# MinghanLi/UniVS

Hardware: AMD Instinct MI355X
Metric: frames/sec per node, 720p T=5 clip, Swin-T 100Q; mask-logit max-abs-err (higher is better)
Workload: dtype f32; 1 GPU; BASELINE config 2: Swin-T UniVS, T=5 @ 720p (736x1280 padded), 100 queries, first clip (no prompt queries); one clip per GPU; frames_per_clip=5, queries=100, parallelism=clip-replicas x1

## Files before the change

### univs_amd/build.py

```python
import os
import shutil
import subprocess
import sys

HERE = os.path.dirname(os.path.abspath(__file__))
CSRC = os.path.join(HERE, "csrc")
LIB = os.path.join(HERE, "libunivs_hip.so")
SOURCES = ["capi.hip", "msda_fwd.hip", "msda_tiled2.hip", "msda_strips.hip", "msda_heads.hip", "msda_bwd.hip", "msda_prepare.hip", "mask_decode.hip", "linear_split.hip", "linear_f16x3.hip", "gemm_f16x3_stream.hip", "gemm_f16x3_tile.hip", "mlp_f16x3.hip", "small_linear.hip", "cross_attn.hip", "window_attn.hip", "window_attn_f16.hip", "resample.hip", "semantic_extract.hip", "layer_norm.hip", "group_norm.hip", "softmax.hip", "proca_attn.hip", "prompt_sampler.hip", "transpose.hip", "mask_stats.hip", "image_post.hip", "video_post.hip", "pair_count.hip", "vss_count.hip", "davis_count.hip", "vis_overlap.hip", "pvos_count.hip", "semantic_decode.hip"]
HEADERS = [os.path.join(CSRC, "common.h"), os.path.join(CSRC, "msda_common.h"), os.path.join(CSRC, "msda_geometry.h"), os.path.join(CSRC, "msda_dev.h"), os.path.join(CSRC, "msda_window_geom.h"), os.path.join(CSRC, "msda_strips_geom.h"), os.path.join(CSRC, "msda_heads_geom.h"), os.path.join(CSRC, "config.h"), os.path.join(CSRC, "window_attn.h"), os.path.join(CSRC, "f16x3.h"), os.path.join(CSRC, "gemm_plan.h"), os.path.join(CSRC, "resample_taps.h"),
           os.path.join(CSRC, "mask_post.h"), os.path.join(CSRC, "count_core.h"), os.path.join(CSRC, "launchers.h"), os.path.join(CSRC, "xattn_merge.h"), os.path.join(CSRC, "skinny_gemm_f32.h"), os.path.join(HERE, "..", "include", "univs_hip.h"),
           os.path.join(HERE, "..", "include", "univs_eval_hip.h"), os.path.join(HERE, "..", "include", "univs_fused_hip.h"),
           os.path.join(HERE, "..", "include", "univs_pvos_hip.h"), os.path.join(HERE, "..", "include", "univs_semantic_hip.h")]


def _hipcc():
    for c in (os.environ.get("HIPCC"), shutil.which("hipcc"), "/opt/rocm/bin/hipcc"):
        if c and os.path.exists(c):
            return c
    raise RuntimeError("hipcc not found (set HIPCC or install ROCm)")


def needs_build():
    if not os.path.exists(LIB):
        return True
    t = os.path.getmtime(LIB)
    deps = [os.path.join(CSRC, s) for s in SOURCES if os.path.exists(os.path.join(CSRC, s))] + HEADERS
    return any(os.path.getmtime(d) > t for d in deps)


def _flags(defines=()):
    return ["--offload-arch=gfx950", "-O3", "-std=c++17", "-fPIC", "-fno-gpu-rdc", "-Wall", "-Wno-unused-function",
            "-I", os.path.join(HERE, "..", "include"), *[f"-D{d}" for d in defines]]


def build(force=False, verbose=True, lib=LIB, defines=(), tag=""):
    if not force and not defines and not needs_build():
        return lib
    from concurrent.futures import ThreadPoolExecutor
    objdir = os.path.join(HERE, "_obj" + tag)
    os.makedirs(objdir, exist_ok=True)
    hipcc = _hipcc()
    hdr_t = max(os.path.getmtime(h) for h in HEADERS)
    srcs = [s for s in SOURCES if os.path.exists(os.path.join(CSRC, s))]

    def compile_one(s):
        src, obj = os.path.join(CSRC, s), os.path.join(objdir, s.replace(".hip", ".o"))
        if not force and os.path.exists(obj) and os.path.getmtime(obj) > max(os.path.getmtime(src), hdr_t):
            return obj
        cmd = [hipcc, *_flags(defines), "-c", src, "-o", obj]
        if verbose:
            print("[univs_amd.build]", " ".join(cmd), file=sys.stderr, flush=True)
        subprocess.run(cmd, check=True)
        return obj

    with ThreadPoolExecutor(max_workers=min(8, os.cpu_count() or 2)) as ex:
        objs = list(ex.map(compile_one, srcs))
    cmd = [hipcc, "--offload-arch=gfx950", "-fPIC", "-shared", "-fno-gpu-rdc", *objs, "-o", lib + ".tmp"]
    if verbose:
        print("[univs_amd.build]", " ".join(cmd), file=sys.stderr, flush=True)
    subprocess.run(cmd, check=True)
    os.replace(lib + ".tmp", lib)
# ... 25 lines not shown
```

### univs_amd/csrc/capi.hip

```cpp
#include <stdarg.h>
#include <string.h>

#include <mutex>

#include "../../include/univs_eval_hip.h"
#include "../../include/univs_fused_hip.h"
#include "../../include/univs_pvos_hip.h"
#include "../../include/univs_semantic_hip.h"
#include "common.h"
#include "config.h"
#include "launchers.h"

namespace univs {

static thread_local char g_err[512] = "";

void set_error(const char* fmt, ...) {
  va_list ap;
  va_start(ap, fmt);
  vsnprintf(g_err, sizeof(g_err), fmt, ap);
  va_end(ap);
}

static void report(const char* name, const char* fmt, va_list ap) {
// ... 45 lines not shown
UnivsConfig config() {
  std::lock_guard<std::mutex> lock(g_cfg_mu);
  return g_cfg;
}
static thread_local int g_msda_last = 0;
static thread_local int g_msda_gen = 0;

static int make_levels(const Entry& e, const int64_t* shapes, const int64_t* starts, int L, int S, LevelTable* lv) {
  if (L < 1 || L > UNIVS_MAX_LEVELS) return e.invalid("num_levels=%d outside [1,%d]", L, UNIVS_MAX_LEVELS);
  if (!shapes || !starts) return e.invalid("spatial_shapes / level_start_index must be host pointers, got NULL");
  int64_t run = 0;
  for (int l = 0; l < L; ++l) {
    const int64_t H = shapes[2 * l], W = shapes[2 * l + 1], st = starts[l];
    if (H <= 0 || W <= 0 || st != run || st + H * W > (int64_t)S)
      return e.invalid("level %d (H=%lld, W=%lld, start=%lld) is inconsistent: expected start=%lld, value length S=%d", l, (long long)H,
                       (long long)W, (long long)st, (long long)run, S);
    run += H * W;
    lv->H[l] = (int)H;
    lv->W[l] = (int)W;
    lv->start[l] = (int)st;
  }
  if (run != (int64_t)S) return e.invalid("the %d levels hold %lld tokens but value has S=%d", L, (long long)run, S);
  for (int l = L; l < UNIVS_MAX_LEVELS; ++l) lv->H[l] = lv->W[l] = lv->start[l] = 0;
  return UNIVS_OK;
}

template <class F>
static int linear_entry(const Entry& e, long long M, int N, int K, int act, const float* residual, bool ptrs_ok, bool resident, F&& launch) {
  if (M < 0 || N < 0 || K < 1 || act < 0 || act > 2 || (act != 0 && residual))
    return e.invalid("bad arguments M=%lld N=%d K=%d act=%d%s", M, N, K, act,
                     (act != 0 && residual) ? " (an activation and a residual exclude each other)" : "");
  if (M == 0 || N == 0) return UNIVS_OK;
  if (!ptrs_ok) return e.null_pointer();
  const int rc = launch(residual ? 3 : act);
  return resident ? e.launched(rc, "shape M=%lld N=%d K=%d (or alignment) is not covered", M, N, K)
                  : e.covered(rc, "shape M=%lld N=%d K=%d (or alignment) is not covered", M, N, K);
}
template <class F>
static int linear_blocked_entry(const Entry& e, long long M, int N, int K, int rows_per_batch, int col_block, bool ptrs_ok, F&& launch) {
  if (M < 0 || N < 1 || K < 1 || rows_per_batch < 1 || col_block < 4 || col_block % 4 != 0 || N % col_block != 0 ||
      (M % rows_per_batch) != 0)
    return e.invalid("bad arguments M=%lld N=%d K=%d rows_per_batch=%d col_block=%d", M, N, K, rows_per_batch, col_block);
  if (M == 0) return UNIVS_OK;
  if (!ptrs_ok) return e.null_pointer();
  return e.launched(launch(), "shape M=%lld N=%d K=%d (or alignment) is not covered (K == 256, M >= 2048)", M, N, K);
}
template <class F>
static int conv_entry(const Entry& e, const char* covers, int T, int Cin, int Cout, int H, int W, bool ptrs_ok, F&& launch) {
  if (T < 0 || Cin < 1 || Cout < 0 || H < 0 || W < 0) return e.invalid("bad dimensions T=%d Cin=%d Cout=%d H=%d W=%d", T, Cin, Cout, H, W);
  if (T == 0 || Cout == 0 || H == 0 || W == 0) return UNIVS_OK;
  if (!ptrs_ok) return e.null_pointer();
  return e.covered(launch(), "T=%d Cin=%d Cout=%d H=%d W=%d not covered (%s)", T, Cin, Cout, H, W, covers);
}

}

using namespace univs;

extern "C" {

const char* univs_version(void) { return "univs_hip 0.1.0 gfx950"; }
const char* univs_last_error(void) { return g_err; }

int univs_configure(const UnivsConfig* cfg) {
  UnivsConfig c = {};
  if (cfg) {
    if (cfg->size < (int)(2 * sizeof(int)) || cfg->size > (int)sizeof(UnivsConfig))
      return invalid_argument(__func__, "UnivsConfig.size=%d (this library: %d)", cfg->size, (int)sizeof(UnivsConfig));
    memcpy(&c, cfg, (size_t)cfg->size);
    if (c.msda_impl < 0 || c.msda_impl > 2 || c.mask_decode_impl < 0 || c.mask_decode_impl > 2 || c.msda_halo > 64 ||
        (c.mask_decode_ct != 0 && c.mask_decode_ct != 2 && c.mask_decode_ct != 4) ||
        (c.linear_terms != 0 && c.linear_terms != 3 && c.linear_terms != 6) || c.mask_decode_wave_tiles > 64)
      return invalid_argument(__func__, "msda_impl=%d mask_decode_impl=%d msda_halo=%d mask_decode_ct=%d linear_terms=%d out of range", c.msda_impl,
                              c.mask_decode_impl, c.msda_halo, c.mask_decode_ct, c.linear_terms);
  }
  c.size = (int)sizeof(UnivsConfig);
  std::lock_guard<std::mutex> lock(g_cfg_mu);
  g_cfg = c;
  return UNIVS_OK;
}

int univs_get_config(UnivsConfig* out) {
  if (!out) return invalid_argument(__func__, "NULL");
  *out = config();
  out->size = (int)sizeof(UnivsConfig);
  return UNIVS_OK;
}

int univs_msda_set_impl(int impl) {
  if (impl < 0 || impl > 2) return invalid_argument(__func__, "impl=%d not in {0,1,2}", impl);
  std::lock_guard<std::mutex> lock(g_cfg_mu);
  g_cfg.msda_impl = impl;
  return UNIVS_OK;
}

int univs_msda_last_impl(void) { return g_msda_last; }
int univs_msda_last_tiled_generation(void) { return g_msda_gen; }

int univs_linear_fused_f32(const float* x, const float* weight, const float* bias, const float* residual, long long M, int N,
                           int K, int act, float* y, void* stream) {
  const Entry e("univs_linear_fused_f32", stream);
  return linear_entry(e, M, N, K, act, residual, x && weight && y, true,
                      [&](int epi) { return linear_split_f32(x, weight, bias, residual, y, M, N, K, epi, e.st); });
}

int univs_presplit_weights_f32(const float* w, int N, int K, int conv, void* wp, float* winv, void* stream) {
  const Entry e("univs_presplit_weights_f32", stream);
  if (N < 0 || K < 32 || K % 32 != 0 || conv < 0 || conv > 2 || (conv == 1 && K % 9 != 0))
    return e.invalid("bad arguments N=%d K=%d mode=%d (K a multiple of 32; mode 1: K = 9 Cin)", N, K, conv);
  if (N == 0) return UNIVS_OK;
  if (!w || !wp || !winv || (reinterpret_cast<uintptr_t>(wp) & 15)) return e.invalid("NULL or unaligned pointer");
  return presplit_f16x3(w, N, K, conv == 1 ? K / 9 : 0, conv == 2 ? 1 : 0, wp, winv, e.st);
}

int univs_conv1x1_presplit_f32(const float* x, const void* wp, const float* winv, const float* bias, int T, int Cin, int Cout, int H,
                               int W, float* y, void* stream) {
  const Entry e("univs_conv1x1_presplit_f32", stream);
  return conv_entry(e, "Cin % 96 or % 128, Cout % 16, >= 4096 pixels", T, Cin, Cout, H, W, x && wp && winv && y,
                    [&] { return conv1x1_f16x3_f32(x, wp, winv, bias, y, T, Cin, Cout, H, W, e.st); });
}

long long univs_cross_attention_workspace(int L, int S, int N, int H) {
  if (L <= 0 || S <= 0 || N <= 0 || H <= 0) return 0;
  return (long long)cross_attention_workspace_floats(L, S, N, H);
}

int univs_cross_attention_f32(const float* q, const float* k, const float* v, const uint8_t* mask, int L, int S, int N, int H, int head_dim,
                              int ldq, int ldk, int ldv, float scale, float* workspace, float* out, void* stream) {
  return univs_cross_attention_flagged_f32(q, k, v, mask, nullptr, 0u, L, S, N, H, head_dim, ldq, ldk, ldv, scale, workspace, out, stream);
}

int univs_cross_attention_flagged_f32(const float* q, const float* k, const float* v, const uint8_t* mask, const uint32_t* mask_row_flags,
                                      uint32_t mask_generation, int L, int S, int N, int H, int head_dim, int ldq, int ldk, int ldv,
                                      float scale, float* workspace, float* out, void* stream) {
  const Entry e("univs_cross_attention_f32", stream);
  if (L < 0 || S < 1 || N < 0 || H < 1 || head_dim < 1) return e.invalid("bad dimensions L=%d S=%d N=%d H=%d head_dim=%d", L, S, N, H, head_dim);
  if (L == 0 || N == 0) return UNIVS_OK;
  if (!q || !k || !v || !workspace || !out || (mask_row_flags && !mask)) return e.invalid("NULL data pointer (row flags come with a mask)");
  return e.covered(cross_attention_f32(q, k, v, mask, mask_row_flags, mask_generation, L, S, N, H, head_dim, ldq, ldk, ldv, scale, workspace,
                                       out, e.st),
                   "L=%d S=%d N=%d H=%d head_dim=%d not covered (head_dim == 32, S >= 32, with a mask S %% 4 == 0, "
                   "N * H <= 65535, 16-byte aligned pointers)", L, S, N, H, head_dim);
}

int univs_mlp_presplit_f32(const float* x, const void* w1p, const float* w1inv, const float* b1, const void* w2p, const float* w2inv,
                           const float* b2, const float* residual, const float* ln_weight, const float* ln_bias, float ln_eps,
                           const float* post_ln_weight, const float* post_ln_bias, float post_ln_eps, const float* post_add,
                           long long post_add_rows, float* y2, long long M, int C, int Hd, int act, float* y, void* stream) {
  return univs_mlp_presplit_v2_f32(x, w1p, w1inv, b1, w2p, w2inv, b2, residual, 0, ln_weight, ln_bias, ln_eps, post_ln_weight, post_ln_bias,
                                   post_ln_eps, post_add, post_add_rows, y2, M, C, Hd, act, y, stream);
}

int univs_mlp_presplit_v2_f32(const float* x, const void* w1p, const float* w1inv, const float* b1, const void* w2p, const float* w2inv,
                              const float* b2, const float* residual, int flags, const float* ln_weight,
                              const float* ln_bias, float ln_eps, const float* post_ln_weight, const float* post_ln_bias, float post_ln_eps,
                              const float* post_add, long long post_add_rows, float* y2, long long M, int C, int Hd, int act, float* y,
                              void* stream) {
  const Entry e("univs_mlp_presplit_f32", stream);
  if (M < 0 || C < 1 || Hd < 1 || (act != 1 && act != 2)) return e.invalid("bad arguments M=%lld C=%d Hd=%d act=%d (1 ReLU, 2 GELU)", M, C, Hd, act);
  if (M == 0) return UNIVS_OK;
  if (!x || !w1p || !w1inv || !w2p || !w2inv || !y) return e.null_pointer();
  if ((flags & ~3) || ((flags & 1) && (residual || !ln_weight || x == y)) || ((flags & 2) && (!post_ln_weight || !y2 || post_add || (flags & 1))))
    return e.invalid("flags=%d: UNIVS_MLP_RESIDUAL_IS_NORMED_X needs ln_weight, no residual pointer and y distinct from x "
                     "(the normalised rows are parked in y); UNIVS_MLP_DUAL_OUTPUT needs post_ln_weight and y2, no post_add, and excludes the other",
                     flags);
  return e.covered(mlp_f16x3_f32(x, w1p, w1inv, b1, w2p, w2inv, b2, residual, ln_weight, ln_bias, ln_eps, post_ln_weight, post_ln_bias,
                                 post_ln_eps, post_add, post_add_rows, y2, y, M, C, Hd, act, flags, e.st),
                   "shape M=%lld C=%d Hd=%d (or alignment) is not covered (C in 96 / 128 / 192 / 256 / 384, Hd %% 32 == 0, M >= 2048)", M, C, Hd);
}

int univs_small_linear_presplit_f32(const float* x, const float* x_add, const void* wp, const float* winv, const float* bias, int n_w,
                                    int f_off, const float* residual, const float* ln_weight, const float* ln_bias, float ln_eps,
// ... 2 lines not shown
  if (M < 0 || N < 0 || K < 1 || n_w < 1 || f_off < 0 || f_off + N > n_w)
    return e.invalid("bad arguments M=%lld N=%d K=%d n_w=%d f_off=%d", M, N, K, n_w, f_off);
  if (M == 0 || N == 0) return UNIVS_OK;
  if (!x || !wp || !winv || !y || (ln_bias && !ln_weight)) return e.null_pointer();
  return e.covered(small_linear_f32(x, x_add, wp, winv, bias, n_w, f_off, residual, ln_weight, ln_bias, ln_eps, y, M, N, K, relu, add_features,
                                    out_T, e.st),
                   "M=%lld N=%d K=%d not covered (K %% 32 == 0, N %% 16 == 0, f_off %% 4 == 0, with a LayerNorm "
                   "N == 256, M <= 1 048 560, 16-byte aligned pointers)", M, N, K);
}

int univs_small_mlp_presplit_f32(const float* x, int stages, const void* const* wp, const float* const* winv, const float* const* bias,
                                 const int* relu, const float* in_ln_weight, const float* in_ln_bias, float in_ln_eps, float* x_normed,
                                 long long M, int out_T, float* y, void* stream) {
  const Entry e("univs_small_mlp_presplit_f32", stream);
  if (M < 0 || stages < 1 || stages > 3 || out_T < 0) return e.invalid("bad arguments M=%lld stages=%d out_T=%d", M, stages, out_T);
  if (M == 0) return UNIVS_OK;
  if (!x || !y || !wp || !winv || !bias || !relu) return e.invalid("NULL pointer");
  return e.covered(small_chain_f32(x, stages, wp, winv, bias, relu, in_ln_weight, in_ln_bias, in_ln_eps, x_normed, y, M, out_T, e.st),
                   "M=%lld not covered (M <= 1 048 560, out_T | M, 16-byte aligned pointers, x_normed / bias only with a LayerNorm)", M);
}

int univs_linear_presplit_f32(const float* x, const void* wp, const float* winv, const float* bias, const float* residual,
                              long long M, int N, int K, int act, float* y, void* stream) {
  const Entry e("univs_linear_presplit_f32", stream);
  return linear_entry(e, M, N, K, act, residual, x && wp && winv && y, false, [&](int epi) {
    int rc = UNIVS_ERR_NOT_IMPLEMENTED;
    if (config().linear_ablate != 6) rc = linear_f16x3_tile_f32(x, wp, winv, bias, residual, y, M, N, K, epi, e.st);
    if (rc == UNIVS_ERR_NOT_IMPLEMENTED) rc = linear_f16x3_stream_f32(x, wp, winv, bias, residual, y, M, N, K, epi, e.st);
    return rc;
  });
}

int univs_linear_resident_presplit_f32(const float* x, const void* wp, const float* winv, const float* bias, const float* residual,
                                       long long M, int N, int K, int act, float* y, void* stream) {
  const Entry e("univs_linear_resident_presplit_f32", stream);
  return linear_entry(e, M, N, K, act, residual, x && wp && winv && y, true, [&](int epi) {
    return linear_split_f32(x, static_cast<const float*>(wp), bias, residual, y, M, N, K, epi, e.st, 0, 0, winv);
  });
}

int univs_linear_blocked_presplit_f32(const float* x, const void* wp, const float* winv, const float* bias, long long M, int N, int K,
                                      int rows_per_batch, int col_block, float* y, void* stream) {
  const Entry e("univs_linear_blocked_presplit_f32", stream);
  return linear_blocked_entry(e, M, N, K, rows_per_batch, col_block, x && wp && winv && y, [&] {
    return linear_split_f32(x, static_cast<const float*>(wp), bias, nullptr, y, M, N, K, 4, e.st, rows_per_batch, col_block,
                            winv);
  });
}

int univs_conv3x3_presplit_f32(const float* x, const void* wp, const float* winv, int T, int Cin, int Cout, int H, int W,
                               float* y, void* stream) {
  const Entry e("univs_conv3x3_presplit_f32", stream);
  return conv_entry(e, "Cin % 128, Cout % 16, >= 4096 pixels", T, Cin, Cout, H, W, x && wp && winv && y,
                    [&] { return conv3x3_f16x3_f32(x, wp, winv, y, T, Cin, Cout, H, W, e.st); });
}

int univs_conv3x3_nhwc_presplit_f32(const float* x, const void* wp, const float* winv, int T, int Cin, int Cout, int H, int W,
                                    float* y, void* stream) {
  const Entry e("univs_conv3x3_nhwc_presplit_f32", stream);
  return conv_entry(e, "Cin % 128, Cout % 16, >= 4096 pixels", T, Cin, Cout, H, W, x && wp && winv && y,
                    [&] { return conv3x3_nhwc_f16x3_f32(x, wp, winv, y, T, Cin, Cout, H, W, e.st); });
}

int univs_conv1x1_fused_presplit_f32(const float* x, int channels_last, const float* affine, const void* wp, const float* winv,
                                     const float* bias, int T, int Cin, int Cout, int H, int W, float* y, void* stream) {
  const Entry e("univs_conv1x1_fused_presplit_f32", stream);
  return conv_entry(e, "Cin % 96 or % 128, Cout % 16, >= 4096 pixels; with an affine H W >= 256 and Cin <= 1024", T, Cin, Cout, H, W,
                    x && wp && winv && y,
                    [&] { return conv1x1_fused_f16x3_f32(x, channels_last, affine, wp, winv, bias, y, T, Cin, Cout, H, W, e.st); });
}

int univs_cross_attention_partials_f32(const float* q, const float* k, const float* v, const uint8_t* mask, const uint32_t* mask_row_flags,
                                       uint32_t mask_generation, int L, int S, int N, int H, int head_dim, int ldq, int ldk, int ldv,
                                       float scale, float* workspace, int* plan, void* stream) {
  const Entry e("univs_cross_attention_partials_f32", stream);
  if (!plan) return e.invalid("NULL plan (a host int)");
  *plan = 0;
  if (L < 0 || S < 1 || N < 0 || H < 1 || head_dim < 1) return e.invalid("bad dimensions L=%d S=%d N=%d H=%d head_dim=%d", L, S, N, H, head_dim);
  if (L == 0 || N == 0) return UNIVS_OK;
  if (!q || !k || !v || !workspace || (mask_row_flags && !mask)) return e.invalid("NULL data pointer (row flags come with a mask)");
  return e.covered(cross_attention_partials_f32(q, k, v, mask, mask_row_flags, mask_generation, L, S, N, H, head_dim, ldq, ldk, ldv, scale,
                                                workspace, plan, e.st),
                   "L=%d S=%d N=%d H=%d head_dim=%d not covered (head_dim == 32, S >= 32, with a mask S %% 4 == 0, "
                   "N * H <= 65535, 16-byte aligned pointers)", L, S, N, H, head_dim);
}

int univs_small_linear_merged_presplit_f32(const float* workspace, long long workspace_floats, int plan, int L, int N, int H, const void* wp,
                                           const float* winv, const float* bias, int n_w, int f_off, const float* residual,
                                           const float* ln_weight, const float* ln_bias, float ln_eps, int n_out, float* y, void* stream) {
  const Entry e("univs_small_linear_merged_presplit_f32", stream);
  const int nseg = plan & 0xffff, nqb = plan >> 16;
  if (L < 0 || N < 0 || H < 1 || n_out < 0 || n_w < 1 || f_off < 0 || f_off + n_out > n_w)
    return e.invalid("bad arguments L=%d N=%d H=%d n_out=%d n_w=%d f_off=%d", L, N, H, n_out, n_w, f_off);
  if (L == 0 || N == 0 || n_out == 0) return UNIVS_OK;
  if (plan <= 0 || nseg < 1 || nqb < 1 || nqb > 7) return e.invalid("plan=%d is not segments + 65536 * query blocks per wave (1 .. 7)", plan);
  const long long chunks = ((long long)L + 16 * nqb - 1) / (16 * nqb);
  const long long need = chunks * N * H * nseg * (16 * nqb) * 34;
  if (workspace_floats < need)
    return e.invalid("workspace of %lld floats, the plan %d of L=%d N=%d H=%d takes %lld", workspace_floats, plan, L, N, H, need);
  if (!workspace || !wp || !winv || !y || (ln_bias && !ln_weight)) return e.null_pointer();
  return e.covered(small_linear_merged_f32(workspace, plan, L, N, H, wp, winv, bias, n_w, f_off, residual, ln_weight, ln_bias, ln_eps, y,
                                           n_out, e.st),
                   "L=%d N=%d H=%d n_out=%d not covered (H <= 8, n_out %% 16 == 0, f_off %% 4 == 0, with a LayerNorm n_out == 256, "
                   "L N <= 1 048 560, 16-byte aligned pointers)", L, N, H, n_out);
}

int univs_patch_embed4_f32(const float* x, const float* weight, const float* bias, const float* ln_weight, const float* ln_bias, float ln_eps,
                           int T, int H, int W, int E, float* out, void* stream) {
  const Entry e("univs_patch_embed4_f32", stream);
  if (T < 0 || H < 0 || W < 0 || E < 1) return e.invalid("bad dimensions T=%d H=%d W=%d E=%d", T, H, W, E);
  if (T == 0 || H == 0 || W == 0) return UNIVS_OK;
  if (!x || !weight || !out) return e.null_pointer();
  return e.covered(patch_embed4_f32(x, weight, bias, ln_weight, ln_bias, ln_eps, out, T, H, W, E, e.st),
                   "T=%d H=%d W=%d E=%d not covered (E in 96 / 128 / 192, H %% 4, W %% 4, 16-byte alignment)", T, H, W, E);
}

int univs_decoder_memory_f32(const float* x, const float* level_embed, const float* pos_yx, const float* pos_t, int T, int C, int HW,
                             float* memory, float* key, void* stream) {
  const Entry e("univs_decoder_memory_f32", stream);
  if (T < 0 || C < 0 || HW < 0) return e.invalid("bad dimensions T=%d C=%d HW=%d", T, C, HW);
  if (T == 0 || C == 0 || HW == 0) return UNIVS_OK;
  if (!x || !level_embed || !pos_yx || !pos_t || !memory || !key) return e.null_pointer();
// ... 618 lines not shown
```

### univs_amd/csrc/gemm_plan.h

```cpp
#pragma once
#include <stddef.h>
#include <stdint.h>

#include <algorithm>

#include "../../include/univs_hip.h"

namespace univs {

constexpr int LS_THREADS = 512;
constexpr int LS_TILE_M = 32;
constexpr int LS_MAX_RB = 7;
constexpr int L3_THREADS = 512;
constexpr int L3_TILE_M = 32;
constexpr int L3_MAX_RB = 8;
constexpr int L3_WPT = 24;
#ifndef UNIVS_GS_THREADS
#define UNIVS_GS_THREADS 512
#endif
constexpr int GS_THREADS = UNIVS_GS_THREADS;
constexpr int GS_TILE_M = 32;
constexpr int GT_THREADS = 512;
enum { EPI_NONE = 0, EPI_RELU = 1, EPI_GELU = 2, EPI_RESIDUAL = 3, EPI_BLOCKED = 4 };

// ... 111 lines not shown
  p.gx = (unsigned)gx;
  p.passes = (unsigned)pp.passes;
  p.rows_per_pass = pp.rows;
  p.remap = cfg.linear_ablate == 5 ? 0 : 1;
  return p;
}

struct TilePlan {
  bool covered;
  int ct, rb, nslot, occ;
  unsigned grid;
  size_t lds;
  int tf, nf;
};
constexpr bool tile_occ2(int ct, int rb) { return (ct == 3 && rb <= 3) || (ct == 4 && rb == 2); }
inline TilePlan plan_tile(long long M, int N, int K, int n_cu, const UnivsConfig& cfg) {
  TilePlan p{};
  if (K % 64 != 0 || K < 384 || N % 4 != 0 || N < 128 || M < 2048 || !fits_int32(M, N) || !fits_int32(M, K) || !fits_int32(K, N)) return p;
  int nslot = K % 128 == 0 ? 4 : K % 96 == 0 ? 3 : 2;
  if (cfg.linear_ablate >= 7 && cfg.linear_ablate <= 9 && K % (32 * (cfg.linear_ablate - 5)) == 0) nslot = cfg.linear_ablate - 5;
  int best_occ = 1;
  double best_t = 1e300;
  for (int ct = 3; ct <= 5; ++ct)
    for (int rb = 2; rb <= 4; ++rb) {
      if (cfg.linear_grid_x >= 3 && cfg.linear_grid_x <= 5 && ct != cfg.linear_grid_x) continue;
      if (cfg.linear_rows_per_pass >= 128 && rb != std::min(4, cfg.linear_rows_per_pass / 64)) continue;
      const int nf = (N + 64 * rb - 1) / (64 * rb);
      int tf = (N + nf - 1) / nf;
      tf = (tf + 3) & ~3;
      if ((tf + 63) / 64 != rb) continue;
      const int occ = tile_occ2(ct, rb) ? 2 : 1;
      const long long wgs = ((M + 32 * ct - 1) / (32 * ct)) * nf;
      const double ks = K / 32;
      const double mfma = 2.0 * ct * rb * 3 * 16;
      const double ldsc = (8.0 * (2 * ct + 2 * rb) * 1024 + 2 * ct * 2048 + tf * 128) / 128.0;
      const double mem = (32.0 * ct * 128 + tf * 128) / 14.0;
      const double t_alone = 1.1 * ks * (std::max(ldsc, mem) + mfma) + 6000.0;
      const double t_full = occ == 2 ? ks * 2.0 * std::max(mfma, std::max(ldsc, mem)) + 6000.0 : t_alone;
      const long long full = wgs / ((long long)n_cu * occ), rem = wgs - full * n_cu * occ;
      const double t = full * t_full + (rem == 0 ? 0.0 : rem > n_cu ? t_full : t_alone);
      if (t < best_t) { best_t = t; p.ct = ct; p.rb = rb; p.nf = nf; p.tf = tf; best_occ = (occ == 2 && wgs > n_cu) ? 2 : 1; }
    }
  if (p.ct == 0) return p;
  if (p.ct == 5 && p.rb == 4 && nslot == 4) nslot = K % 96 == 0 ? 3 : 2;
  if (best_occ == 2) nslot = 2;
  p.covered = true;
  p.nslot = nslot;
  p.occ = best_occ;
  p.grid = (unsigned)(((M + 32 * p.ct - 1) / (32 * p.ct)) * p.nf);
  p.lds = ((size_t)2 * (2 * p.ct * 128) + (size_t)2 * (8 * 64 * p.rb)) * 16 + (size_t)2 * 32 * p.ct * 4 + (size_t)2 * 64 * p.rb * 4;
  return p;
}

}
```

### univs_amd/csrc/launchers.h

```cpp
#pragma once
#include "common.h"

namespace univs {

int msda_forward_generic_f32(const float* value, const LevelTable& lv, const float* loc,
                             const float* attn, int N, int S, int M, int D, int L, int Lq, int P,
                             float* out, hipStream_t st);
int msda_forward_generic_f64(const double* value, const LevelTable& lv, const double* loc,
                             const double* attn, int N, int S, int M, int D, int L, int Lq, int P,
                             double* out, hipStream_t st);

int msda_forward_tiled2_f32(const float* value, const LevelTable& lv, const float* loc, const float* attn, int N,
                            int S, int M, int D, int L, int Lq, int P, float* out, hipStream_t st);

int msda_forward_strips_f32(const float* vhm, const LevelTable& lv, const float* qhm, const float* ref,
                            long long ref_batch_stride, int N, int S, int M, int D, int L, int Lq, int P, float* out,
                            hipStream_t st);

int msda_forward_heads_f32(const float* vhm, const LevelTable& lv, const float* qhm, const float* ref,
                           long long ref_batch_stride, int N, int S, int M, int D, int L, int Lq, int P, float* out,
                           hipStream_t st);

int msda_backward_f32(const float* value, const LevelTable& lv, const float* loc, const float* attn,
                      const float* grad_out, int N, int S, int M, int D, int L, int Lq, int P, float* grad_value,
                      float* grad_loc, float* grad_attn, hipStream_t st);

int msda_prepare_f32(const float* qp, int row_stride, int n_off, const float* ref, long long ref_batch_stride,
                     const LevelTable& lv, int N, int Lq, int M, int L, int P, float* loc, float* attn, hipStream_t st);

int mask_decode_f32(const float* mask_embed, const float* mask_features, int T, int Q, int C,
                    long long HW, float* out, hipStream_t st);
int mask_decode_last_impl();
int mask_decode_attn_f32(const float* mask_embed, const float* feat_lowres, int T, int Q, int C,
                         long long hw, uint8_t* attn_mask, unsigned* row_any_ws, unsigned generation, hipStream_t st);
int attn_mask_rows_reset(uint8_t* attn_mask, const unsigned* row_flags, unsigned generation, long long rows, long long hw, hipStream_t st);

int linear_split_f32(const float* x, const float* w, const float* bias, const float* residual, float* y, long long M, int N,
                     int K, int epi, hipStream_t st, int blk_rows = 0, int blk_cols = 0, const float* winv = nullptr);

int linear_f16x3_f32(const float* x, const float* w, const float* bias, const float* residual, float* y, long long M, int N,
                     int K, int epi, hipStream_t st, int blk_rows, int blk_cols, const float* winv, int n_cu);

int conv3x3_nhwc_f16x3_f32(const float* x, const void* wp, const float* winv, float* y, int T, int Cin, int Cout, int H, int W,
                           hipStream_t st);
int presplit_f16x3(const float* w, int N, int K, int conv_cin, int kperm, void* wp, float* winv, hipStream_t st);
int linear_f16x3_stream_f32(const float* x, const void* wp, const float* winv, const float* bias, const float* residual, float* y,
                            long long M, int N, int K, int epi, hipStream_t st);
int conv3x3_f16x3_f32(const float* x, const void* wp, const float* winv, float* y, int T, int Cin, int Cout, int H, int W,
                      hipStream_t st);
int conv1x1_f16x3_f32(const float* x, const void* wp, const float* winv, const float* bias, float* y, int T, int Cin, int Cout, int H,
                      int W, hipStream_t st);
int conv1x1_fused_f16x3_f32(const float* x, int channels_last, const float* affine, const void* wp, const float* winv, const float* bias,
                            float* y, int T, int Cin, int Cout, int H, int W, hipStream_t st);

int linear_f16x3_tile_f32(const float* x, const void* wp, const float* winv, const float* bias, const float* residual, float* y,
                          long long M, int N, int K, int epi, hipStream_t st);

int mlp_f16x3_f32(const float* x, const void* w1p, const float* w1inv, const float* b1, const void* w2p, const float* w2inv,
                  const float* b2, const float* residual, const float* ln_w, const float* ln_b, float ln_eps, const float* pln_w,
                  const float* pln_b, float pln_eps, const float* post_add, long long post_add_rows, float* y2, float* y, long long M,
                  int C, int Hd, int act, int flags, hipStream_t st);

int small_chain_f32(const float* x, int stages, const void* const* wp, const float* const* winv, const float* const* bias, const int* relu,
                    const float* in_g, const float* in_b, float in_eps, float* xn, float* y, long long M, int out_T, hipStream_t st);
int small_linear_f32(const float* x, const float* xadd, const void* wp, const float* winv, const float* bias, int n_w, int f_off,
                     const float* residual, const float* ln_g, const float* ln_b, float ln_eps, float* y, long long M, int N, int K,
                     int relu, int add_features, int out_T, hipStream_t st);
int small_linear_merged_f32(const float* ws, int plan, int L, int Nb, int Hh, const void* wp, const float* winv, const float* bias, int n_w,
                            int f_off, const float* residual, const float* ln_g, const float* ln_b, float ln_eps, float* y, int N,
                            hipStream_t st);

int cross_attention_f32(const float* q, const float* k, const float* v, const unsigned char* mask, const unsigned* row_flags,
                        unsigned generation, int L, int S, int N, int H, int hd, int ldq, int ldk, int ldv, float scale, float* ws,
                        float* out, hipStream_t st);
int cross_attention_partials_f32(const float* q, const float* k, const float* v, const unsigned char* mask, const unsigned* row_flags,
                                 unsigned generation, int L, int S, int N, int H, int hd, int ldq, int ldk, int ldv, float scale, float* ws,
                                 int* plan_out, hipStream_t st);
size_t cross_attention_workspace_floats(int L, int S, int N, int H);

int window_attention_image_f32(const float* qkv, const float* qkv_bias, const float* bias, const float* shift_mask,
                               int B, int H, int W, int ws, int shift, int nH, int hd, float scale, float* out,
                               hipStream_t st);
int window_attention_f32(const float* qkv, const float* bias, const float* shift_mask, int B_, int nW,
                         int Ntok, int nH, int hd, float scale, float* out, hipStream_t st);

int window_attention_image_f16mma(const float* qkv, const float* qkv_bias, const float* bias, const float* shift_mask, int B,
                                  int H, int W, int ws, int shift, int nH, int hd, float scale, int terms, float* out,
                                  hipStream_t st);

int bilinear_resample_f32(const float* in, const float* addend, float* out, long long planes, int Hin, int Win,
                          int Hout, int Wout, hipStream_t st);
int upsample2x_add_f32(const float* in, const float* addend, const float* affine, float* out, long long planes, int Hin, int Win,
                       hipStream_t st);
int normalize_pad_f32(const float* in, float* out, long long T, int C, int H, int W, int Hp, int Wp, const float* mean, const float* stdv,
                      hipStream_t st);
int bilinear_pyramid3_f32(const float* in, float* out2, float* out4, float* out8, long long planes, int H, int W, hipStream_t st);

int bilinear_crop_nearest_f32(const float* in, float* out, int C, int h, int w, int Hp, int Wp, int Hi, int Wi, int hc, int wc, int t_first,
                              int t_step, int K, hipStream_t st);

int layer_norm_f32(const float* x, const float* res, const float* gamma, const float* beta, long long rows, int C,
                   float eps, float* sum_out, float* out, const float* addend, float* out2, long long addend_rows, hipStream_t st);
int patch_merge_norm_f32(const float* x, const float* gamma, const float* beta, int B, int H, int W, int C, float eps, float* out,
                         hipStream_t st);

int group_norm_affine_f32(const float* x, const float* gamma, const float* beta, int N, int C, long long HW, int groups, float eps,
                          float* ws, long long ws_floats, float* affine, hipStream_t st);
int group_norm_f32(const float* x, const float* gamma, const float* beta, int N, int C, long long HW, int groups,
                   float eps, int relu, float* ws, long long ws_floats, float* out, hipStream_t st);
// ... 70 lines not shown
```

Before: 375.9 frames/s.

## Add tiled MFMA f16x3 conv kernel with fallback to streaming conv

```diff
diff --git a/univs_amd/build.py b/univs_amd/build.py
--- a/univs_amd/build.py
+++ b/univs_amd/build.py
@@ -6,7 +6,7 @@
 HERE = os.path.dirname(os.path.abspath(__file__))
 CSRC = os.path.join(HERE, "csrc")
 LIB = os.path.join(HERE, "libunivs_hip.so")
-SOURCES = ["capi.hip", "msda_fwd.hip", "msda_tiled2.hip", "msda_strips.hip", "msda_heads.hip", "msda_bwd.hip", "msda_prepare.hip", "mask_decode.hip", "linear_split.hip", "linear_f16x3.hip", "gemm_f16x3_stream.hip", "gemm_f16x3_tile.hip", "mlp_f16x3.hip", "small_linear.hip", "cross_attn.hip", "window_attn.hip", "window_attn_f16.hip", "resample.hip", "semantic_extract.hip", "layer_norm.hip", "group_norm.hip", "softmax.hip", "proca_attn.hip", "prompt_sampler.hip", "transpose.hip", "mask_stats.hip", "image_post.hip", "video_post.hip", "pair_count.hip", "vss_count.hip", "davis_count.hip", "vis_overlap.hip", "pvos_count.hip", "semantic_decode.hip"]
+SOURCES = ["capi.hip", "msda_fwd.hip", "msda_tiled2.hip", "msda_strips.hip", "msda_heads.hip", "msda_bwd.hip", "msda_prepare.hip", "mask_decode.hip", "linear_split.hip", "linear_f16x3.hip", "gemm_f16x3_stream.hip", "gemm_f16x3_tile.hip", "conv_f16x3_tile.hip", "mlp_f16x3.hip", "small_linear.hip", "cross_attn.hip", "window_attn.hip", "window_attn_f16.hip", "resample.hip", "semantic_extract.hip", "layer_norm.hip", "group_norm.hip", "softmax.hip", "proca_attn.hip", "prompt_sampler.hip", "transpose.hip", "mask_stats.hip", "image_post.hip", "video_post.hip", "pair_count.hip", "vss_count.hip", "davis_count.hip", "vis_overlap.hip", "pvos_count.hip", "semantic_decode.hip"]
 HEADERS = [os.path.join(CSRC, "common.h"), os.path.join(CSRC, "msda_common.h"), os.path.join(CSRC, "msda_geometry.h"), os.path.join(CSRC, "msda_dev.h"), os.path.join(CSRC, "msda_window_geom.h"), os.path.join(CSRC, "msda_strips_geom.h"), os.path.join(CSRC, "msda_heads_geom.h"), os.path.join(CSRC, "config.h"), os.path.join(CSRC, "window_attn.h"), os.path.join(CSRC, "f16x3.h"), os.path.join(CSRC, "gemm_plan.h"), os.path.join(CSRC, "resample_taps.h"),
            os.path.join(CSRC, "mask_post.h"), os.path.join(CSRC, "count_core.h"), os.path.join(CSRC, "launchers.h"), os.path.join(CSRC, "xattn_merge.h"), os.path.join(CSRC, "skinny_gemm_f32.h"), os.path.join(HERE, "..", "include", "univs_hip.h"),
            os.path.join(HERE, "..", "include", "univs_eval_hip.h"), os.path.join(HERE, "..", "include", "univs_fused_hip.h"),
diff --git a/univs_amd/csrc/capi.hip b/univs_amd/csrc/capi.hip
--- a/univs_amd/csrc/capi.hip
+++ b/univs_amd/csrc/capi.hip
@@ -121,6 +121,10 @@
   if (!ptrs_ok) return e.null_pointer();
   return e.covered(launch(), "T=%d Cin=%d Cout=%d H=%d W=%d not covered (%s)", T, Cin, Cout, H, W, covers);
 }
+template <class F>
+static int tile_else_stream(int rc_tile, F&& stream) {
+  return rc_tile == UNIVS_ERR_NOT_IMPLEMENTED ? stream() : rc_tile;
+}
 
 }
 
@@ -186,7 +190,10 @@
                                int W, float* y, void* stream) {
   const Entry e("univs_conv1x1_presplit_f32", stream);
   return conv_entry(e, "Cin % 96 or % 128, Cout % 16, >= 4096 pixels", T, Cin, Cout, H, W, x && wp && winv && y,
-                    [&] { return conv1x1_f16x3_f32(x, wp, winv, bias, y, T, Cin, Cout, H, W, e.st); });
+                    [&] {
+                      return tile_else_stream(conv_f16x3_tile_f32(x, wp, winv, bias, nullptr, y, T, Cin, Cout, H, W, 1, e.st),
+                                              [&] { return conv1x1_f16x3_f32(x, wp, winv, bias, y, T, Cin, Cout, H, W, e.st); });
+                    });
 }
 
 long long univs_cross_attention_workspace(int L, int S, int N, int H) {
@@ -295,7 +302,10 @@
                                float* y, void* stream) {
   const Entry e("univs_conv3x3_presplit_f32", stream);
   return conv_entry(e, "Cin % 128, Cout % 16, >= 4096 pixels", T, Cin, Cout, H, W, x && wp && winv && y,
-                    [&] { return conv3x3_f16x3_f32(x, wp, winv, y, T, Cin, Cout, H, W, e.st); });
+                    [&] {
+                      return tile_else_stream(conv_f16x3_tile_f32(x, wp, winv, nullptr, nullptr, y, T, Cin, Cout, H, W, 9, e.st),
+                                              [&] { return conv3x3_f16x3_f32(x, wp, winv, y, T, Cin, Cout, H, W, e.st); });
+                    });
 }
 
 int univs_conv3x3_nhwc_presplit_f32(const float* x, const void* wp, const float* winv, int T, int Cin, int Cout, int H, int W,
@@ -310,7 +320,12 @@
   const Entry e("univs_conv1x1_fused_presplit_f32", stream);
   return conv_entry(e, "Cin % 96 or % 128, Cout % 16, >= 4096 pixels; with an affine H W >= 256 and Cin <= 1024", T, Cin, Cout, H, W,
                     x && wp && winv && y,
-                    [&] { return conv1x1_fused_f16x3_f32(x, channels_last, affine, wp, winv, bias, y, T, Cin, Cout, H, W, e.st); });
+                    [&] {
+                      const int rc = channels_last ? UNIVS_ERR_NOT_IMPLEMENTED
+                                                   : conv_f16x3_tile_f32(x, wp, winv, bias, affine, y, T, Cin, Cout, H, W, 1, e.st);
+                      return tile_else_stream(
+                          rc, [&] { return conv1x1_fused_f16x3_f32(x, channels_last, affine, wp, winv, bias, y, T, Cin, Cout, H, W, e.st); });
+                    });
 }
 
 int univs_cross_attention_partials_f32(const float* q, const float* k, const float* v, const uint8_t* mask, const uint32_t* mask_row_flags,
diff --git a/univs_amd/csrc/conv_f16x3_tile.hip b/univs_amd/csrc/conv_f16x3_tile.hip
--- /dev/null
+++ b/univs_amd/csrc/conv_f16x3_tile.hip
@@ -0,0 +1,287 @@
+#include "common.h"
+#include "config.h"
+#include "f16x3.h"
+#include "gemm_plan.h"
+#include "launchers.h"
+
+#include <algorithm>
+#include <cstdlib>
+
+namespace univs {
+
+struct CvArgs {
+  const float* X;
+  const u32x4* Wp;
+  const float* winv;
+  const float* bias;
+  const float* affine;
+  float* Y;
+  int M, N, K;
+  int T, Cin, H, Wd, HW;
+  int ntaps, tap0;
+};
+
+template <int CT, int RB, int NSLOT, int OCC, bool AFF>
+__global__ __launch_bounds__(GT_THREADS, OCC) void conv_f16x3_tile(const CvArgs a) {
+  extern __shared__ __attribute__((aligned(16))) u32x4 lds[];
+  constexpr int NT = 2 * CT;
+  constexpr int TR = 32 * CT;
+  constexpr int TFp = 64 * RB;
+  constexpr int XS = NT * 128;
+  constexpr int WS = 8 * TFp;
+  constexpr int SLOTS = (CT + 7) / 8;
+  u32x4* Xs = lds;
+  u32x4* Ws = lds + 2 * XS;
+  int* Es = reinterpret_cast<int*>(lds + 2 * XS + 2 * WS);
+  float* bias_lds = reinterpret_cast<float*>(Es + 2 * TR);
+  float* winv_lds = bias_lds + TFp;
+  [[maybe_unused]] float* aff_lds = winv_lds + TFp;
+
+  const int row0 = (int)xcd_remap(blockIdx.x, gridDim.x) * TR;
+  const int M = a.M, N = a.N, HW = a.HW, Cin = a.Cin;
+  const int KS = a.K >> 5;
+  const int tid = threadIdx.x, lane = tid & 63;
+  const int wave = __builtin_amdgcn_readfirstlane(tid >> 6);
+  const int j = lane & 15, g = lane >> 4;
+  const int wr = wave >> 2, wf = wave & 3;
+
+  for (int r = tid; r < TFp; r += GT_THREADS) {
+    bias_lds[r] = (a.bias && r < N) ? a.bias[r] : 0.f;
+    winv_lds[r] = r < N ? a.winv[r] : 0.f;
+  }
+  if constexpr (AFF) {
+    const int f0 = row0 / HW, f1 = min(row0 + TR - 1, M - 1) / HW;
+    const int n = (f1 - f0 + 1) * Cin;
+    for (int i = tid; i < n; i += GT_THREADS) {
+      const int f = i < Cin ? f0 : f1, ch = i < Cin ? i : i - Cin;
+      *reinterpret_cast<float2*>(aff_lds + ((f & 1) * Cin + ch) * 2) = *reinterpret_cast<const float2*>(a.affine + ((size_t)f * Cin + ch) * 2);
+    }
+  }
+  __syncthreads();
+
+  const long long planes = (long long)a.T * HW * 4;
+  const __amdgpu_buffer_rsrc_t xrs = __builtin_amdgcn_make_buffer_rsrc(const_cast<float*>(a.X), 0, (int)(planes * Cin), 0x00020000);
+  const __amdgpu_buffer_rsrc_t wrs =
+      __builtin_amdgcn_make_buffer_rsrc(const_cast<u32x4*>(a.Wp), 0, (int)((long long)(a.K >> 3) * 2 * N * 16), 0x00020000);
+  const __amdgpu_buffer_rsrc_t yrs = __builtin_amdgcn_make_buffer_rsrc(a.Y, 0, (int)(planes * N), 0x00020000);
+
+  const int p32 = lane & 31, hh = lane >> 5;
+  unsigned xvo[SLOTS];
+  int py[SLOTS], px[SLOTS];
+  unsigned xdst[SLOTS];
+  [[maybe_unused]] unsigned ao[SLOTS];
+  bool xok[SLOTS];
+  bool rok[SLOTS];
+  int eset[SLOTS];
+  float sx[SLOTS];
+#pragma unroll
+  for (int sl = 0; sl < SLOTS; ++sl) {
+    const int q = wave + 8 * sl;
+    xok[sl] = q < CT;
+    const int mm = row0 + min(q, CT - 1) * 32 + p32;
+    rok[sl] = xok[sl] && mm < M;
+    const int m = min(mm, M - 1);
+    const int f = m / HW, rem = m - f * HW;
+    py[sl] = AFF ? 0 : rem / a.Wd;
+    px[sl] = AFF ? 0 : rem - py[sl] * a.Wd;
+    xvo[sl] = (unsigned)((f * Cin + 16 * hh) * HW + rem) * 4u;
+    ao[sl] = (unsigned)(((f & 1) * Cin + 16 * hh) * 8);
+    xdst[sl] = (unsigned)((2 * min(q, CT - 1) + (p32 >> 4)) * 128 + 2 * hh * 16 + (p32 & 15));
+    eset[sl] = -1000;
+    sx[sl] = 1.0f;
+  }
+  unsigned wvo[RB];
+#pragma unroll
+  for (int v = 0; v < RB; ++v) {
+    const int i = tid + GT_THREADS * v;
+    const int run = i / TFp, rr = i - run * TFp;
+    wvo[v] = rr < N ? (unsigned)((run * N + rr) * 16) : 0xFFFFFFF0u;
+  }
+  const int wstep = 8 * N * 16;
+  f32x4 xq[NSLOT][SLOTS][4];
+  u32x4 wq[NSLOT][RB];
+  int itap = 0, icb = 0, iks = 0;
+  auto issue = [&](int slot) __attribute__((always_inline)) {
+    const int tap = itap + a.tap0;
+    const int dy = tap / 3 - 1, dx = tap - (tap / 3) * 3 - 1;
+#pragma unroll
+    for (int sl = 0; sl < SLOTS; ++sl) {
+      const bool inb = rok[sl] && (AFF || ((unsigned)(py[sl] + dy) < (unsigned)a.H && (unsigned)(px[sl] + dx) < (unsigned)a.Wd));
+      const unsigned vo = inb ? xvo[sl] + (unsigned)((dy * a.Wd + dx) * 4) : 0xFFFFFFF0u;
+#pragma unroll
+      for (int e = 0; e < 16; ++e)
+        xq[slot][sl][e >> 2][e & 3] = __builtin_bit_cast(float, __builtin_amdgcn_raw_buffer_load_b32(xrs, vo, (icb + e) * HW * 4, 0));
+    }
+#pragma unroll
+    for (int v = 0; v < RB; ++v) wq[slot][v] = __builtin_bit_cast(u32x4, __builtin_amdgcn_raw_buffer_load_b128(wrs, wvo[v], iks * wstep, 0));
+    icb += 32;
+    ++iks;
+    if (icb == Cin) {
+      icb = 0;
+      ++itap;
+      if (itap == a.ntaps) {
+        itap = iks = 0;
+#pragma unroll
+        for (int sl = 0; sl < SLOTS; ++sl) rok[sl] = false;
+#pragma unroll
+        for (int v = 0; v < RB; ++v) wvo[v] = 0xFFFFFFF0u;
+      }
+    }
+  };
+  [[maybe_unused]] int cks = 0;
+  auto commit = [&](int slot, int st) __attribute__((always_inline)) {
+#pragma unroll
+    for (int v = 0; v < RB; ++v) Ws[st * WS + tid + GT_THREADS * v] = wq[slot][v];
+#pragma unroll
+    for (int sl = 0; sl < SLOTS; ++sl) {
+      if constexpr (AFF) {
+        const f32x4* ap = reinterpret_cast<const f32x4*>(reinterpret_cast<const char*>(aff_lds) + ao[sl] + (unsigned)(cks * 32 * 8));
+#pragma unroll
+        for (int h = 0; h < 4; ++h) {
+          const f32x4 p0 = ap[2 * h], p1 = ap[2 * h + 1];
+          xq[slot][sl][h][0] = fmaxf(fma_single(xq[slot][sl][h][0], p0[0], p0[1]), 0.f);
+          xq[slot][sl][h][1] = fmaxf(fma_single(xq[slot][sl][h][1], p0[2], p0[3]), 0.f);
+          xq[slot][sl][h][2] = fmaxf(fma_single(xq[slot][sl][h][2], p1[0], p1[1]), 0.f);
+          xq[slot][sl][h][3] = fmaxf(fma_single(xq[slot][sl][h][3], p1[2], p1[3]), 0.f);
+        }
+      }
+      const unsigned mh = max(l3_absmax8(xq[slot][sl][0], xq[slot][sl][1]), l3_absmax8(xq[slot][sl][2], xq[slot][sl][3]));
+      const auto sw = __builtin_amdgcn_permlane32_swap(mh, mh, false, false);
+      const unsigned mk = max(sw[0], sw[1]);
+      const int enew = max(-100, min((int)((mk >> 23) & 255u) - 127, 128));
+      if (enew > eset[sl] + 2) {
+        eset[sl] = enew;
+        sx[sl] = __builtin_bit_cast(float, (unsigned)(127 + 12 - enew) << 23);
+      }
+      f16x8 bh0, bm0, bh1, bm1;
+      l3_split8(xq[slot][sl][0], xq[slot][sl][1], sx[sl], bh0, bm0);
+      l3_split8(xq[slot][sl][2], xq[slot][sl][3], sx[sl], bh1, bm1);
+      if (xok[sl]) {
+        Xs[st * XS + xdst[sl]] = __builtin_bit_cast(u32x4, bh0);
+        Xs[st * XS + xdst[sl] + 64] = __builtin_bit_cast(u32x4, bm0);
+        Xs[st * XS + xdst[sl] + 16] = __builtin_bit_cast(u32x4, bh1);
+        Xs[st * XS + xdst[sl] + 16 + 64] = __builtin_bit_cast(u32x4, bm1);
+        if (hh == 0) Es[st * TR + (wave + 8 * sl) * 32 + p32] = eset[sl];
+      }
+    }
+    if constexpr (AFF) cks = cks + 1 == KS ? 0 : cks + 1;
+  };
+
+  f32x4 acc[RB][CT];
+  int eprev[CT];
+#pragma unroll
+  for (int c = 0; c < CT; ++c) {
+    eprev[c] = -1000;
+#pragma unroll
+    for (int rb = 0; rb < RB; ++rb) acc[rb][c] = (f32x4){0.f, 0.f, 0.f, 0.f};
+  }
+  const int b_unit = (wr * CT) * 128 + g * 16 + j;
+  const int a_unit = (g * 2) * TFp + wf * RB * 16 + j;
+  const int e_idx = wr * CT * 16 + j;
+  auto consume = [&](int st) __attribute__((always_inline)) {
+    int e[CT];
+    bool chg = false;
+#pragma unroll
+    for (int c = 0; c < CT; ++c) {
+      e[c] = Es[st * TR + e_idx + c * 16];
+      chg = chg || e[c] != eprev[c];
+    }
+    if (__builtin_amdgcn_ballot_w64(chg) != 0) {
+#pragma unroll
+      for (int c = 0; c < CT; ++c) {
+        const float ratio = __builtin_bit_cast(float, (unsigned)(127 + max(eprev[c] - e[c], -126)) << 23);
+#pragma unroll
+        for (int rb = 0; rb < RB; ++rb) acc[rb][c] *= ratio;
+        eprev[c] = e[c];
+      }
+    }
+    f16x8 ah[RB], am[RB];
+#pragma unroll
+    for (int rb = 0; rb < RB; ++rb) {
+      ah[rb] = __builtin_bit_cast(f16x8, Ws[st * WS + a_unit + rb * 16]);
+      am[rb] = __builtin_bit_cast(f16x8, Ws[st * WS + a_unit + rb * 16 + TFp]);
+    }
+#pragma unroll
+    for (int c = 0; c < CT; ++c) {
+      const f16x8 bh = __builtin_bit_cast(f16x8, Xs[st * XS + b_unit + c * 128]);
+      const f16x8 bm = __builtin_bit_cast(f16x8, Xs[st * XS + b_unit + c * 128 + 64]);
+#pragma unroll
+      for (int rb = 0; rb < RB; ++rb) acc[rb][c] = __builtin_amdgcn_mfma_f32_16x16x32_f16(am[rb], bh, acc[rb][c], 0, 0, 0);
+#pragma unroll
+      for (int rb = 0; rb < RB; ++rb) acc[rb][c] = __builtin_amdgcn_mfma_f32_16x16x32_f16(ah[rb], bm, acc[rb][c], 0, 0, 0);
+#pragma unroll
+      for (int rb = 0; rb < RB; ++rb) acc[rb][c] = __builtin_amdgcn_mfma_f32_16x16x32_f16(ah[rb], bh, acc[rb][c], 0, 0, 0);
+    }
+  };
+
+#pragma unroll
+  for (int u = 0; u < NSLOT; ++u) issue(u);
+  commit(0, 0);
+#pragma unroll 1
+  for (int s0 = 0; s0 < KS; s0 += NSLOT) {
+#pragma unroll
+    for (int u = 0; u < NSLOT; ++u) {
+      const int s = s0 + u;
+      __syncthreads();
+      issue(u);
+      commit((u + 1) % NSLOT, (s + 1) & 1);
+      consume(s & 1);
+    }
+  }
+
+#pragma unroll
+  for (int c = 0; c < CT; ++c) {
+    const int m = row0 + (wr * CT + c) * 16 + j;
+    const bool row_ok = m < M;
+    const int fr = min(m, M - 1) / HW, rem = min(m, M - 1) - fr * HW;
+    const float sx_inv = __builtin_bit_cast(float, (unsigned)(127 - 12 + eprev[c]) << 23);
+#pragma unroll
+    for (int rb = 0; rb < RB; ++rb) {
+      const int f = (wf * RB + rb) * 16 + 4 * g;
+      const f32x4 wi = *reinterpret_cast<const f32x4*>(winv_lds + f);
+      const f32x4 bi = *reinterpret_cast<const f32x4*>(bias_lds + f);
+      const f32x4 v = (acc[rb][c] * sx_inv) * wi + bi;
+      const unsigned off0 = (row_ok && f < N) ? (unsigned)((fr * N + f) * HW + rem) * 4u : 0xFFFFFFF0u - 3u * (unsigned)HW * 4u;
+      float vx = v.x, vy = v.y, vz = v.z, vw = v.w;
+      asm volatile("" : "+v"(vx), "+v"(vy), "+v"(vz), "+v"(vw));
+      __builtin_amdgcn_raw_buffer_store_b32(__builtin_bit_cast(unsigned, vx), yrs, off0, 0, 0);
+      __builtin_amdgcn_raw_buffer_store_b32(__builtin_bit_cast(unsigned, vy), yrs, off0 + (unsigned)HW * 4u, 0, 0);
+      __builtin_amdgcn_raw_buffer_store_b32(__builtin_bit_cast(unsigned, vz), yrs, off0 + 2u * (unsigned)HW * 4u, 0, 0);
+      __builtin_amdgcn_raw_buffer_store_b32(__builtin_bit_cast(unsigned, vw), yrs, off0 + 3u * (unsigned)HW * 4u, 0, 0);
+    }
+  }
+}
+
+int conv_f16x3_tile_f32(const float* x, const void* wp, const float* winv, const float* bias, const float* affine, float* y, int T, int Cin,
+                        int Cout, int H, int W, int taps, hipStream_t st) {
+  if (T <= 0 || Cout <= 0 || H <= 0 || W <= 0) return UNIVS_OK;
+  const long long HW = (long long)H * W, M = (long long)T * HW;
+  if (!aligned16(x, wp, y, winv, bias) || (reinterpret_cast<uintptr_t>(affine) & 7)) return UNIVS_ERR_NOT_IMPLEMENTED;
+  const ConvTilePlan p = plan_conv_tile(M, HW, Cin, Cout, taps, affine != nullptr, cu_count(), config());
+  if (!p.covered) return UNIVS_ERR_NOT_IMPLEMENTED;
+  CvArgs a{};
+  a.X = x; a.Wp = reinterpret_cast<const u32x4*>(wp); a.winv = winv; a.bias = bias; a.affine = affine; a.Y = y;
+  a.M = (int)M; a.N = Cout; a.K = taps * Cin;
+  a.T = T; a.Cin = Cin; a.H = H; a.Wd = W; a.HW = (int)HW;
+  a.ntaps = taps; a.tap0 = taps == 9 ? 0 : 4;
+  const dim3 grid(p.grid), block(GT_THREADS);
+  const size_t lds = p.lds;
+  bool launched = false;
+#define UNIVS_CV_K(CT_, RB_, NS_, OC_, AFF_)                                                                          \
+  do {                                                                                                                \
+    (void)hipFuncSetAttribute(reinterpret_cast<const void*>(&conv_f16x3_tile<CT_, RB_, NS_, OC_, AFF_>),              \
+                              hipFuncAttributeMaxDynamicSharedMemorySize, (int)lds);                                  \
+    hipLaunchKernelGGL((conv_f16x3_tile<CT_, RB_, NS_, OC_, AFF_>), grid, block, lds, st, a);                         \
+    launched = true;                                                                                                  \
+  } while (0)
+#define UNIVS_CV(CT_, RB_, NS_, OC_, AFF_)                                                                             \
+  if (!launched && p.ct == CT_ && p.rb == RB_ && p.nslot == NS_ && p.occ == OC_ && (affine != nullptr) == AFF_) \
+  UNIVS_CV_K(CT_, RB_, NS_, OC_, AFF_)
+  UNIVS_CONV_TILE_INSTANCES(UNIVS_CV);
+#undef UNIVS_CV
+#undef UNIVS_CV_K
+  if (!launched) return UNIVS_ERR_NOT_IMPLEMENTED;
+  return check_launch("conv_f16x3_tile");
+}
+
+}
diff --git a/univs_amd/csrc/gemm_plan.h b/univs_amd/csrc/gemm_plan.h
--- a/univs_amd/csrc/gemm_plan.h
+++ b/univs_amd/csrc/gemm_plan.h
@@ -187,4 +187,62 @@
   return p;
 }
 
-}
+struct ConvTilePlan {
+  bool covered;
+  int ct, rb, nslot, occ;
+  unsigned grid;
+  size_t lds;
+};
+#define UNIVS_CONV_TILE_INSTANCES(X) \
+  X(4, 4, 2, 1, false);              \
+  X(4, 4, 4, 1, false);              \
+  X(6, 4, 2, 1, false);              \
+  X(8, 4, 2, 1, false);              \
+  X(4, 2, 2, 2, false);              \
+  X(4, 4, 2, 1, true);               \
+  X(4, 4, 4, 1, true);               \
+  X(6, 4, 2, 1, true);               \
+  X(8, 4, 2, 1, true)
+constexpr bool conv_tile_built(int ct, int rb, int nslot, int occ, bool aff) {
+  bool hit = false;
+#define UNIVS_CV_HIT(c, r, n, o, a) hit = hit || (ct == c && rb == r && nslot == n && occ == o && aff == a)
+  UNIVS_CONV_TILE_INSTANCES(UNIVS_CV_HIT);
+#undef UNIVS_CV_HIT
+  return hit;
+}
+constexpr bool conv_tile_occ2(int ct, int rb) { return ct == 4 && rb == 2; }
+constexpr long long CONV_TILE_MIN_M = 32768;
+inline bool conv_tile_preconditions(long long M, long long HW, int Cin, int Cout, int taps, bool affine) {
+  if ((taps != 9 && taps != 1) || Cin < 128 || Cin % 128 != 0 || Cout % 16 != 0 || Cout < 128 || Cout > 256) return false;
+  if (M < 4096 || HW < 1 || M % HW != 0 || !fits_int32(M, std::max(Cin, Cout)) || !fits_int32((long long)taps * Cin, Cout)) return false;
+  return !affine || (taps == 1 && HW >= 256 && Cin <= 1024);
+}
+inline ConvTilePlan plan_conv_tile(long long M, long long HW, int Cin, int Cout, int taps, bool affine, int n_cu, const UnivsConfig& cfg) {
+  ConvTilePlan p{};
+  if (cfg.linear_ablate == 6 || !conv_tile_preconditions(M, HW, Cin, Cout, taps, affine)) return p;
+  const bool forced = cfg.linear_ablate == 11;
+  if (!forced && (M < CONV_TILE_MIN_M || taps != 1)) return p;
+  const int rb = Cout <= 128 ? 2 : 4;
+  const int want_ct = forced ? cfg.linear_grid_x & 15 : 0, want_ns = forced ? (cfg.linear_grid_x >> 4) & 15 : 0;
+  double best_t = 1e300;
+  const double ks = (double)taps * Cin / 32;
+  for (int ct = 2; ct <= 8; ++ct)
+    for (int ns = 2; ns <= 4; ns += 2) {
+      const int occ = conv_tile_occ2(ct, rb) ? 2 : 1;
+      if (!conv_tile_built(ct, rb, ns, occ, affine) || (want_ct && ct != want_ct) || (want_ns && ns != want_ns)) continue;
+      const long long wgs = (M + 32 * ct - 1) / (32 * ct);
+      const double t_wg = (ks * (2300.0 + 130.0 * ct * rb) + 6000.0) * (ns == 4 ? 1.03 : 1.0) * (occ == 2 ? 0.6 : 1.0);
+      const long long rounds = (wgs + (long long)n_cu * occ - 1) / ((long long)n_cu * occ);
+      const double t = rounds * t_wg;
+      if (t < best_t) { best_t = t; p.ct = ct; p.nslot = ns; p.occ = occ; }
+    }
+  if (p.ct == 0) return p;
+  p.covered = true;
+  p.rb = rb;
+  p.grid = (unsigned)((M + 32 * p.ct - 1) / (32 * p.ct));
+  p.lds = ((size_t)2 * (2 * p.ct * 128) + (size_t)2 * (8 * 64 * rb)) * 16 + (size_t)2 * 32 * p.ct * 4 + (size_t)2 * 64 * rb * 4 +
+          (affine ? (size_t)2 * Cin * 8 : 0);
+  return p;
+}
+
+}
diff --git a/univs_amd/csrc/launchers.h b/univs_amd/csrc/launchers.h
--- a/univs_amd/csrc/launchers.h
+++ b/univs_amd/csrc/launchers.h
@@ -55,6 +55,9 @@
 
 int linear_f16x3_tile_f32(const float* x, const void* wp, const float* winv, const float* bias, const float* residual, float* y,
                           long long M, int N, int K, int epi, hipStream_t st);
+
+int conv_f16x3_tile_f32(const float* x, const void* wp, const float* winv, const float* bias, const float* affine, float* y, int T, int Cin,
+                        int Cout, int H, int W, int taps, hipStream_t st);
 
 int mlp_f16x3_f32(const float* x, const void* w1p, const float* w1inv, const float* b1, const void* w2p, const float* w2inv,
                   const float* b2, const float* residual, const float* ln_w, const float* ln_b, float ln_eps, const float* pln_w,
```

Result: no change. 377.0 frames/s, median of 5 (+0.3%).
